# SysCV/sam-pt

Measured on NVIDIA H100. Metric: frames/sec, SAM-PT hot path (PIPS track + SAM ViT encode + prompt/mask decode w/ 12 refinements), higher is better.
Workload: dtype f16 hi.hi + two e4m3 correction passes (~fp32 products) qkv/MLP, f16 hi+lo x3 elsewhere ViT; f32 PIPS + decoder

## Files before the change

### include/sampt_b200.h

```cpp
#ifndef SAMPT_B200_H
#define SAMPT_B200_H
#include <stddef.h>
#include <stdint.h>

#ifdef __cplusplus
extern "C" {
#endif

typedef struct sampt_ctx sampt_ctx;

#define SAMPT_F32 0
#define SAMPT_F16 1
#define SAMPT_U8 2
#define SAMPT_I32 3
#define SAMPT_BF16 4

const char* sampt_last_error(void);
int sampt_version(void);
int sampt_ctx_create(int device, sampt_ctx** out);
int sampt_ctx_destroy(sampt_ctx* ctx);
int sampt_ctx_set_workspace(sampt_ctx* ctx, void* dev_ptr, size_t bytes);
int sampt_ctx_set_vit_workspace(sampt_ctx* ctx, void* dev_ptr, size_t bytes);
int sampt_ctx_set_decoder_workspace(sampt_ctx* ctx, void* dev_ptr, size_t bytes);
int sampt_set_tensor(sampt_ctx* ctx, const char* name, void* dev_ptr, int dtype, int ndim, const int64_t* dims);
int sampt_unset_tensors(sampt_ctx* ctx, const char* prefix);
long long sampt_launch_count(sampt_ctx* ctx);

int sampt_pips_fnet(sampt_ctx* ctx, const uint8_t* frames_u8, int T, int H, int W, int stride, float* fmaps, void* stream);
int sampt_pips_pyramid(sampt_ctx* ctx, const float* fmaps, int T, int H4, int W4, float* l1, float* l2, float* l3,
                       void* stream);
int sampt_pips_track(sampt_ctx* ctx, const float* fmaps, const float* l1, const float* l2, const float* l3, int T, int H4,
                     int W4, const float* query_points, int N, int S, int stride, float thr0, int iters, int flip,
                     int max_windows, float* traj, float* vis, void* stream);
int sampt_pips_window(sampt_ctx* ctx, const float* fmaps, const float* l1, const float* l2, const float* l3, int H4, int W4,
                      const float* xys, const float* coords_init, const float* feat_init, int N, int S, int stride, int iters,
                      float* coords_out, float* vis_e, float* ffeat_out, void* stream);
int sampt_pips_corr_lookup(sampt_ctx* ctx, const float* fmaps, const float* l1, const float* l2, const float* l3, int S,
                           int H4, int W4, const float* ffeats, const float* coords, int N, float* fcorr, void* stream);

int sampt_linear_f32(sampt_ctx* ctx, const float* X, int ldx, const float* W, int ldw, const float* bias,
                     const float* residual, int ldr, float* Y, int ldy, int M, int N, int K, int act, void* stream);

int sampt_gemm_f16(sampt_ctx* ctx, const void* A, int lda, const void* B, int ldb, int M, int N, int K, int precision,
                   int is_bf16, const float* bias, int act, void* out16, float* out32, const float* resid, int ldc,
                   int split_off, void* stream);

int sampt_gemm_f8c(sampt_ctx* ctx, const void* A, const void* B, int M, int N, int K, const float* acc_scale_dev, const float* bias,
                   int act, void* out16, float* out32, const float* resid, int ldc, int split_off, int out_f8, void* stream);
int sampt_split_f8c(sampt_ctx* ctx, const float* x, int M, int K, void* out, void* stream);

int sampt_attention_f16(sampt_ctx* ctx, const void* Qx, const void* Kx, const void* Vt, int BH, int Lq, int Lk, int Lkp, int DK,
                        int HD, int NT, int nheads, void* out, int ld_out, int split_off, void* stream);

int sampt_test_gemm_tc(sampt_ctx* ctx, const void* A, int lda, const void* B, int ldb, int M, int N, int K, int nseg,
                       const int* a_off_host, const int* b_off_host, const int* f8_host, const float* bias, int act, int is_bf16,
                       void* out16, float* out32, const float* resid, int resid_mod, const int* rowmap, const int* skip,
                       const float* acc_scale, int ldc, int split_off, int out_f8, void* stream);
int sampt_test_vit_attention(sampt_ctx* ctx, const void* qkv, const float* rel_pos_h, const float* rel_pos_w, int nwb, int nheads,
                             int S, int D, int DK, int Lkp, void* Qx, void* Kx, void* Vt, void* out, int ld_out, int split_off,
                             int out_f8, void* stream);
int sampt_test_vit_embed(sampt_ctx* ctx, const void* image, int is_f32, int B, int Hr, int Wr, int embed_dim, int img_size,
                         int patch_size, int precision, const float* mean3, const float* std3, void* a_out, float* x_out,
                         void* stream);
int sampt_test_vit_ln(sampt_ctx* ctx, const float* x, int ldx, const int* src, int M, int D, int normalize, const float* gamma,
                      const float* beta, int layout, void* out, void* stream);
int sampt_test_vit_block(sampt_ctx* ctx, int blk, int is_global, float* x, float* x_mid, int B, int Hr, int Wr, int live_only,
                         int embed_dim, int num_heads, int window_size, int img_size, int patch_size, int precision, void* stream);
int sampt_test_vit_neck(sampt_ctx* ctx, const float* x, int B, int embed_dim, int img_size, int patch_size, int out_chans,
                        int precision, float* features, void* stream);
int sampt_test_sam_attention(sampt_ctx* ctx, int kind, const float* q, const float* k, const float* v, float* out, int T, int Nk,
                             void* stream);
int sampt_test_sam_prompt(sampt_ctx* ctx, const float* feat_tok, int G, const float* coords, const int* labels, int K, const float* box,
                          const float* mask_in, float* tokens_out, float* src_out, void* stream);
int sampt_test_sam_upscale(sampt_ctx* ctx, const float* u1, const float* hyper, int n_masks, int G, float* low_res, float* u_out,
                           void* stream);
int sampt_test_sam_postprocess(sampt_ctx* ctx, const float* low_res, int n_masks, int G, int in_h, int in_w, int H, int W, float* out,
                               int* bbox5, float* box4, int* skip, int* n_done, void* stream);
int sampt_test_pips_conv(sampt_ctx* ctx, const char* name, int tc, const void* in, int is_f32, int Nimg, int H, int W, int Cin,
                         int Cout, int R, int stride, int pad, float* out, void* stream);
int sampt_test_pips_inorm(sampt_ctx* ctx, const float* x, const float* res, int mode, int Nimg, int HW, int C, float* y, float* stats,
                          float* res_stats, void* stream);
int sampt_test_pips_resize(sampt_ctx* ctx, const float* in, int Nimg, int Hi, int Wi, int C, float* out, int Ho, int Wo, int Ctot,
                           int coff, void* stream);
int sampt_test_pips_corr(sampt_ctx* ctx, const float* fmaps, const float* l1, const float* l2, const float* l3, int H4, int W4,
                         const float* ffeats, const float* coords, int N, int S, const uint8_t* active_host, int f, int n_missing,
                         const int* slots_host, float* xin, void* stream);
int sampt_test_pips_window_op(sampt_ctx* ctx, int op, int N, int S, int T, int stride, int f, int n_missing, const int* slots_host,
                              const uint8_t* active_host, const float* fmaps, int H4, int W4, float* coords, float* ffeats,
                              float* feat_init, float* traj, float* vis, int* cur, float* x, float* xln, int layer,
                              const float* delta, float thr0, void* stream);
int sampt_test_cotracker_input(sampt_ctx* ctx, const float* fmaps, const float* l1, const float* l2, const float* l3, int H4, int W4,
                               const int* slots_host, const float* coords, const float* ffeats, const float* track_mask,
                               const float* vis_init, const float* time_emb, int N, float* pos, float* xin, void* stream);
int sampt_test_cotracker_ln(sampt_ctx* ctx, int op, const float* x, int M, int K, float* y32, void* y16, void* stream);
int sampt_test_cotracker_attn(sampt_ctx* ctx, const float* qkv, float* out, int G, int L, int gstride, int lstride, int qsplit,
                              void* stream);
int sampt_test_cotracker_block(sampt_ctx* ctx, int kind, int blk, int tc, float* x, int N, void* stream);
int sampt_test_cotracker_update(sampt_ctx* ctx, const float* delta, float* coords, float* ffeats, int N, float* vis_out, void* stream);

int sampt_pil_resize_u8(sampt_ctx* ctx, const uint8_t* in, int B, int H, int W, int Ho, int Wo, const int* hbounds,
                        const int* hcoef, int hksize, const int* vbounds, const int* vcoef, int vksize, uint8_t* tmp,
                        uint8_t* out, void* stream);
int sampt_vit_encode(sampt_ctx* ctx, const uint8_t* resized_u8, int B, int Hr, int Wr, int depth, int embed_dim, int num_heads,
                     int window_size, const int* global_idx_host, int n_global, int img_size, int patch_size, int out_chans,
                     int precision, const float* pixel_mean_host, const float* pixel_std_host, float* features, float* interm,
                     void* stream);

int sampt_sam_features_to_tokens(sampt_ctx* ctx, const float* feat_nchw, float* feat_tok, int C, int GG, void* stream);
int sampt_sam_predict(sampt_ctx* ctx, const float* feat_tok, int G, const float* coords, const int* labels, int K,
                      const float* box, const float* mask_input, int multimask, int in_h, int in_w, int H, int W, float* logits,
// ... 74 lines not shown
```

### sam-pt_b200/csrc/decoder.cu

```cuda
#include <cstdlib>

#include "common.cuh"
#include "kernels.cuh"
#include "tc_api.cuh"
#include "../../include/sampt_b200.h"

namespace sampt {

#define SKIP_RETURN(skip) \
  if ((skip) != nullptr && *(skip) != 0) return;

struct PromptArgs {
  const float* coords;
  const int* labels;
  int K;
  const float* box;
  int use_box;
  const float* gauss;
  const float* pt_emb[4];
  const float* not_a_point;
  const float* out_tokens;
  int n_out_tok;
  float img_size;
};
// ... 729 lines not shown
    SAMPT_TRY(get_f32(c, md + "embedding_encoder.1.weight", &w->enc_lnw)); SAMPT_TRY(get_f32(c, md + "embedding_encoder.1.bias", &w->enc_lnb));
    SAMPT_TRY(get_f32(c, md + "embedding_encoder.3.weight", &w->enc3_w)); SAMPT_TRY(get_f32(c, md + "embedding_encoder.3.bias", &w->enc3_b));
    SAMPT_TRY(get_f32(c, md + "compress_vit_feat.0.weight_gemm", &w->cv0_w)); SAMPT_TRY(get_f32(c, md + "compress_vit_feat.0.bias4", &w->cv0_b4));
    SAMPT_TRY(get_f32(c, md + "compress_vit_feat.1.weight", &w->cv_lnw)); SAMPT_TRY(get_f32(c, md + "compress_vit_feat.1.bias", &w->cv_lnb));
    SAMPT_TRY(get_f32(c, md + "compress_vit_feat.3.weight", &w->cv3_w)); SAMPT_TRY(get_f32(c, md + "compress_vit_feat.3.bias", &w->cv3_b));
    w->vit_dim = (int)c->find(md + "compress_vit_feat.0.weight_gemm")->dims[1];
  }
  return 0;
}

struct DecBufs {
  float *tokens, *queries, *qpe, *tq, *tk, *tv, *ta, *tmp, *mlp_h;
  float *src, *keys, *ik, *iv, *iq, *ia;
  __half *keys16 = nullptr, *ia16 = nullptr;
  float *u1, *hyper, *iou4, *part;
  float *u_sam, *mf1, *mf2;
  int T;
};

#define LAUNCH_OK() do { c->launches++; SAMPT_LAUNCH_CHECK(); } while (0)

static int sg(Ctx* c, cudaStream_t st, const float* X, int ldx, const float* W, const float* b, const float* resid, int ldr,
              float* Y, int ldy, int M, int N, int K, int act, const int* skip) {
  return sgemm_nt_skip(c, st, X, ldx, W, K, b, resid, ldr, Y, ldy, M, N, K, act, skip);
}

__global__ void __launch_bounds__(256)
split_f32_kernel(const float* __restrict__ x, __half* __restrict__ out, long long n4 , int K, const int* skip) {
  SKIP_RETURN(skip);
  const long long i = (long long)blockIdx.x * 256 + threadIdx.x;
  if (i >= n4) return;
  const long long e = i * 4;
  const long long r = e / K;
  const int cidx = (int)(e % K);
  const float4 v = *reinterpret_cast<const float4*>(x + e);
  const __half2 h0 = __floats2half2_rn(v.x, v.y), h1 = __floats2half2_rn(v.z, v.w);
  const float2 f0 = __half22float2(h0), f1 = __half22float2(h1);
  const __half2 l0 = __floats2half2_rn(v.x - f0.x, v.y - f0.y), l1 = __floats2half2_rn(v.z - f1.x, v.w - f1.y);
  __half* o = out + r * 2 * K + cidx;
  *reinterpret_cast<uint2*>(o) = make_uint2(*reinterpret_cast<const uint32_t*>(&h0), *reinterpret_cast<const uint32_t*>(&h1));
  *reinterpret_cast<uint2*>(o + K) = make_uint2(*reinterpret_cast<const uint32_t*>(&l0), *reinterpret_cast<const uint32_t*>(&l1));
}
static int split_rows(Ctx* c, cudaStream_t st, const float* x, __half* out, int rows, int K, const int* skip) {
  const long long n4 = (long long)rows * K / 4;
  split_f32_kernel<<<cdiv(n4, 256), 256, 0, st>>>(x, out, n4, K, skip);
  c->launches++;
  SAMPT_LAUNCH_CHECK();
  return 0;
}
static int tcg(Ctx* c, cudaStream_t st, const __half* X16, const __half* W16, const float* b, const float* resid, float* Y, int ldy,
               int M, int N, int K, const int* skip) {
  GemmSeg seg{};
  seg.nseg = 3;
  seg.a_off[0] = 0; seg.b_off[0] = 0;
  seg.a_off[1] = K; seg.b_off[1] = 0;
  seg.a_off[2] = 0; seg.b_off[2] = K;
  GemmEpi ep{};
  ep.out32 = Y; ep.ldc = ldy; ep.bias = b; ep.resid = resid; ep.skip = skip;
  return gemm_tc(c, st, X16, 2 * K, W16, 2 * K, M, N, K, seg, ep);
}

static int launch_tok_self(Ctx* c, cudaStream_t st, int kind, const float* q, const float* k, const float* v, float* out, int T,
                           const int* skip) {
  if (kind == 1) {
    const size_t smem = ((size_t)2 * T * 33 + (size_t)8 * T + 8 * 32) * sizeof(float);
    SAMPT_CHECK(smem <= 200 * 1024, "too many prompt tokens (%d) for the token self-attention", T);
    SAMPT_TRY(ensure_func_smem(c, "attn_tok_self_kernel<32>", attn_tok_self_kernel<32>, 200 * 1024));
    attn_tok_self_kernel<32><<<dim3(cdiv(T, 32), 8), 256, smem, st>>>(q, k, v, out, T, 8, skip);
  } else {
    attn_q_small_kernel<32><<<dim3(T, 8), 256, 0, st>>>(q, k, v, out, T, 8, skip);
  }
  LAUNCH_OK();
  return 0;
}
static int launch_t2i(Ctx* c, cudaStream_t st, const float* q, const float* k, const float* v, float* part, float* out, int T, int Nk,
                      const int* skip) {
  constexpr int KPS = 256;
  const int nsplit = (Nk + KPS - 1) / KPS;
  attn_t2i_partial_kernel<16, KPS><<<dim3(nsplit, 8), 256, 0, st>>>(q, k, v, part, T, Nk, 8, skip);
  LAUNCH_OK();
  attn_t2i_combine_kernel<16><<<cdiv(T * 128, 128), 128, 0, st>>>(part, out, T, 8, nsplit, skip);
  LAUNCH_OK();
  return 0;
}
static int launch_i2t(Ctx* c, cudaStream_t st, const float* q, const float* k, const float* v, float* out, int N, int T, const int* skip) {
  attn_kv_small_kernel<16><<<cdiv((long long)cdiv(N, 32) * 8, 8), 256, 0, st>>>(q, k, v, out, N, T, 8, skip);
  LAUNCH_OK();
  return 0;
}

static int attn_tok_to_img(Ctx* c, cudaStream_t st, const AttnW& a, const float* q_in, const float* keys, const float* pek,
                           DecBufs& b, float* out , const float* resid, int GG, const int* skip) {
  const int T = b.T;
  SAMPT_TRY(sg(c, st, q_in, 256, a.qw, a.qb, nullptr, 0, b.tq, 128, T, 128, 256, 0, skip));
  if (a.kw16 != nullptr) {
    SAMPT_TRY(tcg(c, st, b.keys16, a.kw16, a.kb, pek, b.ik, 128, GG, 128, 256, skip));
    SAMPT_TRY(tcg(c, st, b.keys16, a.vw16, a.vb, nullptr, b.iv, 128, GG, 128, 256, skip));
  } else {
    SAMPT_TRY(sg(c, st, keys, 256, a.kw, a.kb, pek, 128, b.ik, 128, GG, 128, 256, 0, skip));
    SAMPT_TRY(sg(c, st, keys, 256, a.vw, a.vb, nullptr, 0, b.iv, 128, GG, 128, 256, 0, skip));
  }
  SAMPT_TRY(launch_t2i(c, st, b.tq, b.ik, b.iv, b.part, b.ta, T, GG, skip));
  SAMPT_TRY(sg(c, st, b.ta, 128, a.ow, a.ob, resid, 256, out, 256, T, 256, 128, 0, skip));
  return 0;
}

static int two_way_layer(Ctx* c, cudaStream_t st, const LayerW& L, int idx, DecBufs& b, int GG, const int* skip) {
  const int T = b.T;
  if (idx == 0) {
// ... 493 lines not shown
```

### sam-pt_b200/csrc/gemm_tc.cu

```cuda
#include "common.cuh"
#include "tc_common.cuh"
#include "kernels.cuh"
#include "tc_api.cuh"
#include "../../include/sampt_b200.h"

namespace sampt {

using namespace tc;

constexpr int G_BM = 128, G_BN = 128, G_BK = 64, G_STAGES = 3;
constexpr int G_A_BYTES = G_BM * G_BK * 2;
constexpr int G_B_BYTES = G_BN * G_BK * 2;
constexpr int G_STAGE_BYTES = G_A_BYTES + G_B_BYTES;
constexpr int G_SMEM_BYTES = G_STAGES * G_STAGE_BYTES + 1024  + 256 ;
constexpr int G_THREADS = 288;

__global__ void __launch_bounds__(G_THREADS, 2)
gemm_tc_kernel(const __grid_constant__ CUtensorMap tmA, const __grid_constant__ CUtensorMap tmB, int M, int N, int K,
               GemmSeg seg, GemmEpi ep) {
  if (ep.skip != nullptr && *ep.skip != 0) return;
  extern __shared__ uint8_t smem_raw[];
  uint8_t* smem = reinterpret_cast<uint8_t*>((reinterpret_cast<uintptr_t>(smem_raw) + 1023) & ~uintptr_t(1023));
  uint64_t* full_bar = reinterpret_cast<uint64_t*>(smem + G_STAGES * G_STAGE_BYTES);
  uint64_t* empty_bar = full_bar + G_STAGES;

  const int warp = threadIdx.x >> 5, lane = threadIdx.x & 31;
  const int n_tiles = (N + G_BN - 1) / G_BN;
  const int m_blk = blockIdx.x / n_tiles, n_blk = blockIdx.x % n_tiles;
  int seg_kb[3];
#pragma unroll
  for (int i = 0; i < 3; ++i) seg_kb[i] = i < seg.nseg ? (seg.f8[i] ? K / (2 * G_BK) : K / G_BK) : 0;

  if (threadIdx.x == 0) {
    for (int i = 0; i < G_STAGES; ++i) { mbar_init(&full_bar[i], 1); mbar_init(&empty_bar[i], 256); }
    fence_barrier_init();
  }
  __syncthreads();

  if (warp == 8) {
    if (lane == 0) {
      tma_prefetch_desc(&tmA);
      tma_prefetch_desc(&tmB);
      uint32_t it = 0;
      for (int sg = 0; sg < seg.nseg; ++sg) {
        for (int kb = 0; kb < seg_kb[sg]; ++kb, ++it) {
          const int s = it % G_STAGES;
          const uint32_t ph = (it / G_STAGES) & 1;
          mbar_wait(&empty_bar[s], ph ^ 1);
          const int kk = kb * G_BK;
          uint8_t* sa = smem + s * G_STAGE_BYTES;
          mbar_expect_tx(&full_bar[s], G_STAGE_BYTES);
          tma_load_2d(sa, &tmA, &full_bar[s], seg.a_off[sg] + kk, m_blk * G_BM);
          tma_load_2d(sa + G_A_BYTES, &tmB, &full_bar[s], seg.b_off[sg] + kk, n_blk * G_BN);
        }
      }
    }
    return;
  }

  const int g = warp >> 2, w = warp & 3;
  float acc[64];
#pragma unroll
  for (int i = 0; i < 64; ++i) acc[i] = 0.f;
  uint32_t it = 0;
  int prev_s = -1;
  for (int sg = 0; sg < seg.nseg; ++sg) {
    const bool f8 = seg.f8[sg] != 0;
    for (int kb = 0; kb < seg_kb[sg]; ++kb, ++it) {
      const int s = it % G_STAGES;
      mbar_wait(&full_bar[s], (it / G_STAGES) & 1);
      const uint32_t sa = smem_u32(smem + s * G_STAGE_BYTES);
      const uint64_t adesc = make_smem_desc_sw128(sa + g * 64 * 128);
      const uint64_t bdesc = make_smem_desc_sw128(sa + G_A_BYTES);
      wgmma_fence();
      if (f8) {
#pragma unroll
        for (int k = 0; k < 4; ++k) wgmma_m64n128k32_e4m3(acc, adesc + (uint64_t)(2 * k), bdesc + (uint64_t)(2 * k));
      } else if (ep.is_bf16) {
#pragma unroll
        for (int k = 0; k < 4; ++k) wgmma_m64n128k16_bf16(acc, adesc + (uint64_t)(2 * k), bdesc + (uint64_t)(2 * k));
      } else {
#pragma unroll
        for (int k = 0; k < 4; ++k) wgmma_m64n128k16_f16(acc, adesc + (uint64_t)(2 * k), bdesc + (uint64_t)(2 * k));
      }
      wgmma_commit();
      wgmma_wait<1>();
      if (prev_s >= 0) mbar_arrive(&empty_bar[prev_s]);
      prev_s = s;
    }
  }
  wgmma_wait<0>();
  wgmma_fence_regs(acc);

  const float acc_scale = ep.acc_scale ? __ldg(ep.acc_scale) : 1.0f;
  const int c2 = 2 * (lane & 3);
#pragma unroll
  for (int h = 0; h < 2; ++h) {
    const int m = m_blk * G_BM + g * 64 + w * 16 + (lane >> 2) + 8 * h;
    if (m >= M) continue;
    long long drow = m;
    if (ep.rowmap) drow = ep.rowmap[m];
    if (drow < 0) continue;
#pragma unroll
    for (int i = 0; i < G_BN / 8; ++i) {
      const int n = n_blk * G_BN + 8 * i + c2;
      if (n >= N) continue;
      float v0 = acc[4 * i + 2 * h], v1 = acc[4 * i + 2 * h + 1];
      v0 *= acc_scale; v1 *= acc_scale;
      if (ep.bias) { v0 += __ldg(ep.bias + n); v1 += __ldg(ep.bias + n + 1); }
      if (ep.act == 1) { v0 = gelu_erf(v0); v1 = gelu_erf(v1); }
      else if (ep.act == 3) { v0 = gelu_tanh(v0); v1 = gelu_tanh(v1); }
      if (ep.out32) {
        float* o = ep.out32 + (size_t)drow * ep.ldc + n;
        if (ep.resid) {
          const long long rrow = ep.resid_mod > 0 ? (drow % ep.resid_mod) : drow;
          const float2 t = *reinterpret_cast<const float2*>(ep.resid + (size_t)rrow * ep.ldc + n);
          v0 += t.x; v1 += t.y;
        }
        *reinterpret_cast<float2*>(o) = make_float2(v0, v1);
      } else if (ep.is_bf16) {
        *reinterpret_cast<__nv_bfloat162*>(ep.out16 + (size_t)drow * ep.ldc + n) = __floats2bfloat162_rn(v0, v1);
      } else {
        __half* o = ep.out16 + (size_t)drow * ep.ldc + n;
        const __half2 hv = __floats2half2_rn(v0, v1);
        *reinterpret_cast<__half2*>(o) = hv;
        const float2 hf = __half22float2(hv);
        if (ep.split_off > 0 && ep.out_f8) {
          uint8_t* ob = reinterpret_cast<uint8_t*>(ep.out16 + (size_t)drow * ep.ldc + ep.split_off) + n;
          uint16_t l8, h8;
          asm("cvt.rn.satfinite.e4m3x2.f32 %0, %1, %2;" : "=h"(l8) : "f"((v1 - hf.y) * F8_LO_SCALE), "f"((v0 - hf.x) * F8_LO_SCALE));
          asm("cvt.rn.satfinite.e4m3x2.f32 %0, %1, %2;" : "=h"(h8) : "f"(v1 * F8_HI_SCALE), "f"(v0 * F8_HI_SCALE));
          *reinterpret_cast<uint16_t*>(ob) = l8;
          *reinterpret_cast<uint16_t*>(ob + ep.split_off) = h8;
        } else if (ep.split_off > 0) {
          *reinterpret_cast<__half2*>(o + ep.split_off) = __floats2half2_rn(v0 - hf.x, v1 - hf.y);
        }
      }
    }
  }
}

bool gemm_f8c_applicable(int M, int N, int K) { return M >= 256 && N % 256 == 0 && K % (2 * G_BK) == 0; }

int gemm_tc(Ctx* c, cudaStream_t st, const void* A, int lda, const void* B, int ldb, int M, int N, int K, const GemmSeg& seg,
            const GemmEpi& ep) {
  SAMPT_CHECK(K % G_BK == 0 && K > 0, "gemm_tc: K (%d) must be a positive multiple of %d", K, G_BK);
  SAMPT_CHECK(N % 32 == 0, "gemm_tc: N (%d) must be a multiple of 32", N);
  SAMPT_CHECK(seg.nseg >= 1 && seg.nseg <= 3, "gemm_tc: nseg out of range");
  SAMPT_CHECK((ep.out16 != nullptr) != (ep.out32 != nullptr), "gemm_tc: exactly one of out16/out32 must be set");
  SAMPT_CHECK(ep.ldc % 8 == 0, "gemm_tc: ldc must be a multiple of 8");
  SAMPT_CHECK(ep.act == 0 || ep.act == 1 || ep.act == 3, "gemm_tc: act %d is not 0 (none), 1 (GELU erf) or 3 (GELU tanh)", ep.act);
  const bool f8 = (seg.f8[0] | seg.f8[1] | seg.f8[2]) != 0;
  SAMPT_CHECK(!f8 || K % (2 * G_BK) == 0, "gemm_tc: e4m3 segments need K %% 128 == 0 (K = %d)", K);
  SAMPT_CHECK(!f8 || !ep.is_bf16, "gemm_tc: e4m3 segments go with fp16 operands");
  CUtensorMap tmA, tmB;
  SAMPT_TRY(make_tmap_2d_f16(&tmA, A, (uint64_t)lda, (uint64_t)M, (uint64_t)lda * 2, G_BK, G_BM));
  SAMPT_TRY(make_tmap_2d_f16(&tmB, B, (uint64_t)ldb, (uint64_t)N, (uint64_t)ldb * 2, G_BK, G_BN));
  const int m_tiles = (M + G_BM - 1) / G_BM, n_tiles = (N + G_BN - 1) / G_BN;
  const int grid = m_tiles * n_tiles;
  GemmSeg ord{};
  ord.nseg = seg.nseg;
  int j = 0;
  for (int pass = 1; pass >= 0; --pass)
    for (int i = 0; i < seg.nseg; ++i)
      if ((seg.f8[i] != 0) == (pass == 1)) { ord.a_off[j] = seg.a_off[i]; ord.b_off[j] = seg.b_off[i]; ord.f8[j] = seg.f8[i]; ++j; }
  SAMPT_TRY(ensure_func_smem(c, "gemm_tc_kernel", gemm_tc_kernel, G_SMEM_BYTES));
  gemm_tc_kernel<<<grid, G_THREADS, G_SMEM_BYTES, st>>>(tmA, tmB, M, N, K, ord, ep);
  c->launches++;
  SAMPT_LAUNCH_CHECK();
  return 0;
}

}

using namespace sampt;

extern "C" int sampt_gemm_f16(sampt_ctx* ctx, const void* A, int lda, const void* B, int ldb, int M, int N, int K, int precision,
                              int is_bf16, const float* bias, int act, void* out16, float* out32, const float* resid, int ldc,
                              int split_off, void* stream) {
  Ctx* c = reinterpret_cast<Ctx*>(ctx);
  GemmSeg seg{};
  seg.nseg = precision;
  SAMPT_CHECK(precision >= 1 && precision <= 3, "precision must be 1, 2 or 3");
  if (precision == 2) {
    seg.a_off[0] = 0; seg.b_off[0] = 0;
    seg.a_off[1] = 0; seg.b_off[1] = K;
  } else {
    seg.a_off[0] = 0; seg.b_off[0] = 0;
    seg.a_off[1] = K; seg.b_off[1] = 0;
    seg.a_off[2] = 0; seg.b_off[2] = K;
  }
  GemmEpi ep{};
  ep.out16 = reinterpret_cast<__half*>(out16);
  ep.out32 = out32;
  ep.resid = resid;
  ep.bias = bias;
  ep.rowmap = nullptr;
  ep.ldc = ldc;
  ep.act = act;
  ep.split_off = split_off;
  ep.is_bf16 = is_bf16;
  return gemm_tc(c, reinterpret_cast<cudaStream_t>(stream), A, lda, B, ldb, M, N, K, seg, ep);
}

extern "C" int sampt_gemm_f8c(sampt_ctx* ctx, const void* A, const void* B, int M, int N, int K, const float* acc_scale_dev,
                              const float* bias, int act, void* out16, float* out32, const float* resid, int ldc, int split_off,
                              int out_f8, void* stream) {
  Ctx* c = reinterpret_cast<Ctx*>(ctx);
  SAMPT_CHECK(gemm_f8c_applicable(M, N, K), "sampt_gemm_f8c: needs M >= 256, N %% 256 == 0, K %% 128 == 0 (got %d x %d x %d)", M, N, K);
  GemmEpi ep{};
  ep.out16 = reinterpret_cast<__half*>(out16);
  ep.out32 = out32;
  ep.resid = resid;
  ep.bias = bias;
  ep.ldc = ldc;
  ep.act = act;
  ep.split_off = split_off;
  ep.out_f8 = out_f8;
  ep.acc_scale = acc_scale_dev;
  return gemm_tc(c, reinterpret_cast<cudaStream_t>(stream), A, 2 * K, B, 2 * K, M, N, K, make_seg_f8(K), ep);
}

extern "C" int sampt_test_gemm_tc(sampt_ctx* ctx, const void* A, int lda, const void* B, int ldb, int M, int N, int K, int nseg,
                                  const int* a_off_host, const int* b_off_host, const int* f8_host, const float* bias, int act,
                                  int is_bf16, void* out16, float* out32, const float* resid, int resid_mod, const int* rowmap,
                                  const int* skip, const float* acc_scale, int ldc, int split_off, int out_f8, void* stream) {
  SAMPT_CHECK(nseg >= 1 && nseg <= 3, "sampt_test_gemm_tc: nseg %d out of range", nseg);
  GemmSeg seg{};
  seg.nseg = nseg;
  for (int i = 0; i < nseg; ++i) { seg.a_off[i] = a_off_host[i]; seg.b_off[i] = b_off_host[i]; seg.f8[i] = f8_host[i]; }
  GemmEpi ep{};
  ep.out16 = reinterpret_cast<__half*>(out16);
  ep.out32 = out32;
  ep.resid = resid;
  ep.bias = bias;
  ep.rowmap = rowmap;
  ep.ldc = ldc;
  ep.act = act;
  ep.split_off = split_off;
  ep.is_bf16 = is_bf16;
  ep.resid_mod = resid_mod;
  ep.skip = skip;
  ep.acc_scale = acc_scale;
  ep.out_f8 = out_f8;
  return gemm_tc(reinterpret_cast<Ctx*>(ctx), reinterpret_cast<cudaStream_t>(stream), A, lda, B, ldb, M, N, K, seg, ep);
}

extern "C" int sampt_split_f8c(sampt_ctx* ctx, const float* x, int M, int K, void* out, void* stream) {
  Ctx* c = reinterpret_cast<Ctx*>(ctx);
  return ln_rows(c, reinterpret_cast<cudaStream_t>(stream), x, K, nullptr, nullptr, nullptr, 0.f, reinterpret_cast<__half*>(out), 2 * K, K,
                 M, K, 0, 1);
}
```

### sam-pt_b200/csrc/tc_common.cuh

```cuda
#pragma once
#include <cuda.h>
#include <cuda_runtime.h>
#include <cstdint>

namespace sampt {
namespace tc {

__device__ __forceinline__ uint32_t smem_u32(const void* p) { return (uint32_t)__cvta_generic_to_shared(p); }

__device__ __forceinline__ void mbar_init(uint64_t* bar, uint32_t count) {
  asm volatile("mbarrier.init.shared::cta.b64 [%0], %1;" ::"r"(smem_u32(bar)), "r"(count));
}
__device__ __forceinline__ void fence_barrier_init() { asm volatile("fence.mbarrier_init.release.cluster;" ::: "memory"); }
__device__ __forceinline__ void fence_proxy_async() { asm volatile("fence.proxy.async.shared::cta;" ::: "memory"); }
__device__ __forceinline__ void mbar_expect_tx(uint64_t* bar, uint32_t bytes) {
  asm volatile("mbarrier.arrive.expect_tx.shared::cta.b64 _, [%0], %1;" ::"r"(smem_u32(bar)), "r"(bytes) : "memory");
}
__device__ __forceinline__ void mbar_arrive(uint64_t* bar) {
  asm volatile("mbarrier.arrive.shared::cta.b64 _, [%0];" ::"r"(smem_u32(bar)) : "memory");
}
__device__ __forceinline__ uint32_t mbar_try_wait(uint64_t* bar, uint32_t parity) {
  uint32_t ok;
  asm volatile(
      "{\n"
      ".reg .pred p;\n"
      "mbarrier.try_wait.parity.shared::cta.b64 p, [%1], %2;\n"
      "selp.b32 %0, 1, 0, p;\n"
      "}\n"
      : "=r"(ok)
      : "r"(smem_u32(bar)), "r"(parity)
      : "memory");
  return ok;
}
__device__ __forceinline__ void mbar_wait(uint64_t* bar, uint32_t parity) {
  while (!mbar_try_wait(bar, parity)) {
  }
}

__device__ __forceinline__ void tma_prefetch_desc(const CUtensorMap* m) {
  asm volatile("prefetch.tensormap [%0];" ::"l"(reinterpret_cast<uint64_t>(m)) : "memory");
}
__device__ __forceinline__ void tma_load_2d(void* smem_dst, const CUtensorMap* m, uint64_t* bar, int c0, int c1) {
  asm volatile(
      "cp.async.bulk.tensor.2d.shared::cluster.global.mbarrier::complete_tx::bytes [%0], [%1, {%3, %4}], [%2];" ::"r"(
          smem_u32(smem_dst)),
      "l"(reinterpret_cast<uint64_t>(m)), "r"(smem_u32(bar)), "r"(c0), "r"(c1)
      : "memory");
}
__device__ __forceinline__ void tma_load_3d(void* smem_dst, const CUtensorMap* m, uint64_t* bar, int c0, int c1, int c2) {
  asm volatile(
      "cp.async.bulk.tensor.3d.shared::cluster.global.mbarrier::complete_tx::bytes [%0], [%1, {%3, %4, %5}], [%2];" ::"r"(
          smem_u32(smem_dst)),
      "l"(reinterpret_cast<uint64_t>(m)), "r"(smem_u32(bar)), "r"(c0), "r"(c1), "r"(c2)
      : "memory");
}

__device__ __forceinline__ void wgmma_fence() { asm volatile("wgmma.fence.sync.aligned;" ::: "memory"); }
__device__ __forceinline__ void wgmma_commit() { asm volatile("wgmma.commit_group.sync.aligned;" ::: "memory"); }
template <int N>
__device__ __forceinline__ void wgmma_wait() { asm volatile("wgmma.wait_group.sync.aligned %0;" ::"n"(N) : "memory"); }
template <int R>
__device__ __forceinline__ void wgmma_fence_regs(float (&d)[R]) {
#pragma unroll
  for (int i = 0; i < R; ++i) asm volatile("" : "+f"(d[i])::"memory");
}

__device__ __forceinline__ void wgmma_m64n128k16_f16(float (&d)[64], uint64_t da, uint64_t db) {
  asm volatile(
      "{\n.reg .pred p;\nsetp.ne.b32 p, %66, 0;\n"
      "wgmma.mma_async.sync.aligned.m64n128k16.f32.f16.f16 {%0, %1, %2, %3, %4, %5, %6, %7, %8, %9, %10, %11, %12, %13, %14, %15, %16, %17, %18, %19, %20, %21, %22, %23, %24, %25, %26, %27, %28, %29, %30, %31, %32, %33, %34, %35, %36, %37, %38, %39, %40, %41, %42, %43, %44, %45, %46, %47, %48, %49, %50, %51, %52, %53, %54, %55, %56, %57, %58, %59, %60, %61, %62, %63}, %64, %65, p, 1, 1, 0, 0;\n}\n"
      : "+f"(d[0]), "+f"(d[1]), "+f"(d[2]), "+f"(d[3]), "+f"(d[4]), "+f"(d[5]), "+f"(d[6]), "+f"(d[7]), "+f"(d[8]), "+f"(d[9]), "+f"(d[10]), "+f"(d[11]), "+f"(d[12]), "+f"(d[13]), "+f"(d[14]), "+f"(d[15]), "+f"(d[16]), "+f"(d[17]), "+f"(d[18]), "+f"(d[19]), "+f"(d[20]), "+f"(d[21]), "+f"(d[22]), "+f"(d[23]), "+f"(d[24]), "+f"(d[25]), "+f"(d[26]), "+f"(d[27]), "+f"(d[28]), "+f"(d[29]), "+f"(d[30]), "+f"(d[31]), "+f"(d[32]), "+f"(d[33]), "+f"(d[34]), "+f"(d[35]), "+f"(d[36]), "+f"(d[37]), "+f"(d[38]), "+f"(d[39]), "+f"(d[40]), "+f"(d[41]), "+f"(d[42]), "+f"(d[43]), "+f"(d[44]), "+f"(d[45]), "+f"(d[46]), "+f"(d[47]), "+f"(d[48]), "+f"(d[49]), "+f"(d[50]), "+f"(d[51]), "+f"(d[52]), "+f"(d[53]), "+f"(d[54]), "+f"(d[55]), "+f"(d[56]), "+f"(d[57]), "+f"(d[58]), "+f"(d[59]), "+f"(d[60]), "+f"(d[61]), "+f"(d[62]), "+f"(d[63])
      : "l"(da), "l"(db), "r"(1));
}

__device__ __forceinline__ void wgmma_m64n128k16_bf16(float (&d)[64], uint64_t da, uint64_t db) {
  asm volatile(
      "{\n.reg .pred p;\nsetp.ne.b32 p, %66, 0;\n"
      "wgmma.mma_async.sync.aligned.m64n128k16.f32.bf16.bf16 {%0, %1, %2, %3, %4, %5, %6, %7, %8, %9, %10, %11, %12, %13, %14, %15, %16, %17, %18, %19, %20, %21, %22, %23, %24, %25, %26, %27, %28, %29, %30, %31, %32, %33, %34, %35, %36, %37, %38, %39, %40, %41, %42, %43, %44, %45, %46, %47, %48, %49, %50, %51, %52, %53, %54, %55, %56, %57, %58, %59, %60, %61, %62, %63}, %64, %65, p, 1, 1, 0, 0;\n}\n"
      : "+f"(d[0]), "+f"(d[1]), "+f"(d[2]), "+f"(d[3]), "+f"(d[4]), "+f"(d[5]), "+f"(d[6]), "+f"(d[7]), "+f"(d[8]), "+f"(d[9]), "+f"(d[10]), "+f"(d[11]), "+f"(d[12]), "+f"(d[13]), "+f"(d[14]), "+f"(d[15]), "+f"(d[16]), "+f"(d[17]), "+f"(d[18]), "+f"(d[19]), "+f"(d[20]), "+f"(d[21]), "+f"(d[22]), "+f"(d[23]), "+f"(d[24]), "+f"(d[25]), "+f"(d[26]), "+f"(d[27]), "+f"(d[28]), "+f"(d[29]), "+f"(d[30]), "+f"(d[31]), "+f"(d[32]), "+f"(d[33]), "+f"(d[34]), "+f"(d[35]), "+f"(d[36]), "+f"(d[37]), "+f"(d[38]), "+f"(d[39]), "+f"(d[40]), "+f"(d[41]), "+f"(d[42]), "+f"(d[43]), "+f"(d[44]), "+f"(d[45]), "+f"(d[46]), "+f"(d[47]), "+f"(d[48]), "+f"(d[49]), "+f"(d[50]), "+f"(d[51]), "+f"(d[52]), "+f"(d[53]), "+f"(d[54]), "+f"(d[55]), "+f"(d[56]), "+f"(d[57]), "+f"(d[58]), "+f"(d[59]), "+f"(d[60]), "+f"(d[61]), "+f"(d[62]), "+f"(d[63])
      : "l"(da), "l"(db), "r"(1));
}

__device__ __forceinline__ void wgmma_m64n128k32_e4m3(float (&d)[64], uint64_t da, uint64_t db) {
  asm volatile(
      "{\n.reg .pred p;\nsetp.ne.b32 p, %66, 0;\n"
      "wgmma.mma_async.sync.aligned.m64n128k32.f32.e4m3.e4m3 {%0, %1, %2, %3, %4, %5, %6, %7, %8, %9, %10, %11, %12, %13, %14, %15, %16, %17, %18, %19, %20, %21, %22, %23, %24, %25, %26, %27, %28, %29, %30, %31, %32, %33, %34, %35, %36, %37, %38, %39, %40, %41, %42, %43, %44, %45, %46, %47, %48, %49, %50, %51, %52, %53, %54, %55, %56, %57, %58, %59, %60, %61, %62, %63}, %64, %65, p, 1, 1;\n}\n"
      : "+f"(d[0]), "+f"(d[1]), "+f"(d[2]), "+f"(d[3]), "+f"(d[4]), "+f"(d[5]), "+f"(d[6]), "+f"(d[7]), "+f"(d[8]), "+f"(d[9]), "+f"(d[10]), "+f"(d[11]), "+f"(d[12]), "+f"(d[13]), "+f"(d[14]), "+f"(d[15]), "+f"(d[16]), "+f"(d[17]), "+f"(d[18]), "+f"(d[19]), "+f"(d[20]), "+f"(d[21]), "+f"(d[22]), "+f"(d[23]), "+f"(d[24]), "+f"(d[25]), "+f"(d[26]), "+f"(d[27]), "+f"(d[28]), "+f"(d[29]), "+f"(d[30]), "+f"(d[31]), "+f"(d[32]), "+f"(d[33]), "+f"(d[34]), "+f"(d[35]), "+f"(d[36]), "+f"(d[37]), "+f"(d[38]), "+f"(d[39]), "+f"(d[40]), "+f"(d[41]), "+f"(d[42]), "+f"(d[43]), "+f"(d[44]), "+f"(d[45]), "+f"(d[46]), "+f"(d[47]), "+f"(d[48]), "+f"(d[49]), "+f"(d[50]), "+f"(d[51]), "+f"(d[52]), "+f"(d[53]), "+f"(d[54]), "+f"(d[55]), "+f"(d[56]), "+f"(d[57]), "+f"(d[58]), "+f"(d[59]), "+f"(d[60]), "+f"(d[61]), "+f"(d[62]), "+f"(d[63])
      : "l"(da), "l"(db), "r"(1));
}

// ... 71 lines not shown
```

Before: 23.85.

## Make tensor-core GEMM persistent with ping-pong consumer warpgroups and deeper pipeline

Converts the TMA+wgmma GEMM into a persistent kernel whose grid is capped at the SM count. Two consumer warpgroups alternate whole 128x128 tiles using named barriers, so one warpgroup's epilogue overlaps the other's MMA. When a CTA owns only one tile, the old split across row halves is kept. The pipeline deepens from 3 to 7 stages at one CTA per SM, and the decoder's 3-segment hi/lo order is changed to put the small correction terms first. This aims to hide epilogue cost and cut wave-quantization and launch tail, at the cost of occupancy and more register pressure from the two 64-float accumulators.

```diff
diff --git a/include/sampt_b200.h b/include/sampt_b200.h
--- a/include/sampt_b200.h
+++ b/include/sampt_b200.h
@@ -56,6 +56,11 @@
                        const int* a_off_host, const int* b_off_host, const int* f8_host, const float* bias, int act, int is_bf16,
                        void* out16, float* out32, const float* resid, int resid_mod, const int* rowmap, const int* skip,
                        const float* acc_scale, int ldc, int split_off, int out_f8, void* stream);
+int sampt_test_gemm_tc_grid(sampt_ctx* ctx, const void* A, int lda, const void* B, int ldb, int M, int N, int K, int nseg,
+                            const int* a_off_host, const int* b_off_host, const int* f8_host, const float* bias, int act,
+                            int is_bf16, void* out16, float* out32, const float* resid, int resid_mod, const int* rowmap,
+                            const int* skip, const float* acc_scale, int ldc, int split_off, int out_f8, int max_ctas,
+                            void* stream);
 int sampt_test_vit_attention(sampt_ctx* ctx, const void* qkv, const float* rel_pos_h, const float* rel_pos_w, int nwb, int nheads,
                              int S, int D, int DK, int Lkp, void* Qx, void* Kx, void* Vt, void* out, int ld_out, int split_off,
                              int out_f8, void* stream);
diff --git a/sam-pt_b200/csrc/decoder.cu b/sam-pt_b200/csrc/decoder.cu
--- a/sam-pt_b200/csrc/decoder.cu
+++ b/sam-pt_b200/csrc/decoder.cu
@@ -805,9 +805,9 @@
                int M, int N, int K, const int* skip) {
   GemmSeg seg{};
   seg.nseg = 3;
-  seg.a_off[0] = 0; seg.b_off[0] = 0;
-  seg.a_off[1] = K; seg.b_off[1] = 0;
-  seg.a_off[2] = 0; seg.b_off[2] = K;
+  seg.a_off[0] = K; seg.b_off[0] = 0;
+  seg.a_off[1] = 0; seg.b_off[1] = K;
+  seg.a_off[2] = 0; seg.b_off[2] = 0;
   GemmEpi ep{};
   ep.out32 = Y; ep.ldc = ldy; ep.bias = b; ep.resid = resid; ep.skip = skip;
   return gemm_tc(c, st, X16, 2 * K, W16, 2 * K, M, N, K, seg, ep);
diff --git a/sam-pt_b200/csrc/gemm_tc.cu b/sam-pt_b200/csrc/gemm_tc.cu
--- a/sam-pt_b200/csrc/gemm_tc.cu
+++ b/sam-pt_b200/csrc/gemm_tc.cu
@@ -8,14 +8,144 @@
 
 using namespace tc;
 
-constexpr int G_BM = 128, G_BN = 128, G_BK = 64, G_STAGES = 3;
+constexpr int G_BM = 128, G_BN = 128, G_BK = 64, G_STAGES = 7;
 constexpr int G_A_BYTES = G_BM * G_BK * 2;
 constexpr int G_B_BYTES = G_BN * G_BK * 2;
 constexpr int G_STAGE_BYTES = G_A_BYTES + G_B_BYTES;
 constexpr int G_SMEM_BYTES = G_STAGES * G_STAGE_BYTES + 1024  + 256 ;
-constexpr int G_THREADS = 288;
-
-__global__ void __launch_bounds__(G_THREADS, 2)
+constexpr int G_THREADS = 384;
+constexpr int G_BAR_MMA = 1;
+
+template <int NH>
+__device__ __forceinline__ void gemm_tile_mma(float (&acc)[NH][64], uint8_t* smem, uint64_t* full_bar, uint64_t* empty_bar,
+                                              uint32_t it, const int (&seg_kb)[3], int nseg, const GemmSeg& seg, bool is_bf16,
+                                              int row64, int handoff) {
+#pragma unroll
+  for (int h = 0; h < NH; ++h)
+#pragma unroll
+    for (int i = 0; i < 64; ++i) acc[h][i] = 0.f;
+  int prev_s = -1;
+  for (int sg = 0; sg < nseg; ++sg) {
+    const bool f8 = seg.f8[sg] != 0;
+    for (int kb = 0; kb < seg_kb[sg]; ++kb, ++it) {
+      const int s = it % G_STAGES;
+      mbar_wait(&full_bar[s], (it / G_STAGES) & 1);
+      const uint32_t sa = smem_u32(smem + s * G_STAGE_BYTES);
+      const uint64_t bdesc = make_smem_desc_sw128(sa + G_A_BYTES);
+      uint64_t adesc[NH];
+#pragma unroll
+      for (int h = 0; h < NH; ++h) adesc[h] = make_smem_desc_sw128(sa + (row64 + h) * 64 * 128);
+      wgmma_fence();
+      if (f8) {
+#pragma unroll
+        for (int k = 0; k < 4; ++k)
+#pragma unroll
+          for (int h = 0; h < NH; ++h) wgmma_m64n128k32_e4m3(acc[h], adesc[h] + (uint64_t)(2 * k), bdesc + (uint64_t)(2 * k));
+      } else if (is_bf16) {
+#pragma unroll
+        for (int k = 0; k < 4; ++k)
+#pragma unroll
+          for (int h = 0; h < NH; ++h) wgmma_m64n128k16_bf16(acc[h], adesc[h] + (uint64_t)(2 * k), bdesc + (uint64_t)(2 * k));
+      } else {
+#pragma unroll
+        for (int k = 0; k < 4; ++k)
+#pragma unroll
+          for (int h = 0; h < NH; ++h) wgmma_m64n128k16_f16(acc[h], adesc[h] + (uint64_t)(2 * k), bdesc + (uint64_t)(2 * k));
+      }
+      wgmma_commit();
+      wgmma_wait<1>();
+      if (prev_s >= 0) mbar_arrive(&empty_bar[prev_s]);
+      prev_s = s;
+    }
+  }
+  if (handoff >= 0) named_bar_arrive(handoff, 256);
+  wgmma_wait<0>();
+  mbar_arrive(&empty_bar[prev_s]);
+#pragma unroll
+  for (int h = 0; h < NH; ++h) wgmma_fence_regs(acc[h]);
+}
+
+enum { EPI_F32 = 0, EPI_F16 = 1, EPI_F16_SPLIT = 2, EPI_F16_F8 = 3, EPI_BF16 = 4 };
+
+template <int OUT, int ACT>
+__device__ __forceinline__ void gemm_tile_store(const float (&acc)[64], int m64, int n0, int M, int N, const GemmEpi& ep,
+                                                float acc_scale) {
+  const int w = (threadIdx.x >> 5) & 3, lane = threadIdx.x & 31;
+  const int c2 = 2 * (lane & 3);
+#pragma unroll
+  for (int h = 0; h < 2; ++h) {
+    const int m = m64 + w * 16 + (lane >> 2) + 8 * h;
+    if (m >= M) continue;
+    long long drow = m;
+    if (ep.rowmap) drow = ep.rowmap[m];
+    if (drow < 0) continue;
+#pragma unroll
+    for (int i = 0; i < G_BN / 8; ++i) {
+      const int n = n0 + 8 * i + c2;
+      if (n >= N) continue;
+      float v0 = acc[4 * i + 2 * h], v1 = acc[4 * i + 2 * h + 1];
+      v0 *= acc_scale; v1 *= acc_scale;
+      if (ep.bias) { v0 += __ldg(ep.bias + n); v1 += __ldg(ep.bias + n + 1); }
+      if constexpr (ACT == 1) { v0 = gelu_erf(v0); v1 = gelu_erf(v1); }
+      else if constexpr (ACT == 3) { v0 = gelu_tanh(v0); v1 = gelu_tanh(v1); }
+      if constexpr (OUT == EPI_F32) {
+        float* o = ep.out32 + (size_t)drow * ep.ldc + n;
+        if (ep.resid) {
+          const long long rrow = ep.resid_mod > 0 ? (drow % ep.resid_mod) : drow;
+          const float2 t = *reinterpret_cast<const float2*>(ep.resid + (size_t)rrow * ep.ldc + n);
+          v0 += t.x; v1 += t.y;
+        }
+        *reinterpret_cast<float2*>(o) = make_float2(v0, v1);
+      } else if constexpr (OUT == EPI_BF16) {
+        *reinterpret_cast<__nv_bfloat162*>(ep.out16 + (size_t)drow * ep.ldc + n) = __floats2bfloat162_rn(v0, v1);
+      } else {
+        __half* o = ep.out16 + (size_t)drow * ep.ldc + n;
+        const __half2 hv = __floats2half2_rn(v0, v1);
+        *reinterpret_cast<__half2*>(o) = hv;
+        const float2 hf = __half22float2(hv);
+        if constexpr (OUT == EPI_F16_F8) {
+          uint8_t* ob = reinterpret_cast<uint8_t*>(ep.out16 + (size_t)drow * ep.ldc + ep.split_off) + n;
+          uint16_t l8, h8;
+          asm("cvt.rn.satfinite.e4m3x2.f32 %0, %1, %2;" : "=h"(l8) : "f"((v1 - hf.y) * F8_LO_SCALE), "f"((v0 - hf.x) * F8_LO_SCALE));
+          asm("cvt.rn.satfinite.e4m3x2.f32 %0, %1, %2;" : "=h"(h8) : "f"(v1 * F8_HI_SCALE), "f"(v0 * F8_HI_SCALE));
+          *reinterpret_cast<uint16_t*>(ob) = l8;
+          *reinterpret_cast<uint16_t*>(ob + ep.split_off) = h8;
+        } else if constexpr (OUT == EPI_F16_SPLIT) {
+          *reinterpret_cast<__half2*>(o + ep.split_off) = __floats2half2_rn(v0 - hf.x, v1 - hf.y);
+        }
+      }
+    }
+  }
+}
+
+template <int OUT, int ACT, int NH>
+__device__ __forceinline__ void gemm_tile_store_rows(const float (&acc)[NH][64], int m0, int n0, int M, int N, const GemmEpi& ep,
+                                                     float acc_scale) {
+#pragma unroll
+  for (int h = 0; h < NH; ++h) gemm_tile_store<OUT, ACT>(acc[h], m0 + 64 * h, n0, M, N, ep, acc_scale);
+}
+
+template <int NH>
+__device__ __forceinline__ void gemm_tile_epilogue(const float (&acc)[NH][64], int m0, int n0, int M, int N, const GemmEpi& ep,
+                                                   float acc_scale) {
+  const int out = ep.out32 ? EPI_F32 : ep.is_bf16 ? EPI_BF16 : ep.split_off <= 0 ? EPI_F16 : ep.out_f8 ? EPI_F16_F8 : EPI_F16_SPLIT;
+#define GEMM_EPI_CASE(O)                                                                              \
+  case O:                                                                                             \
+    if (ep.act == 1) gemm_tile_store_rows<O, 1, NH>(acc, m0, n0, M, N, ep, acc_scale);               \
+    else if (ep.act == 3) gemm_tile_store_rows<O, 3, NH>(acc, m0, n0, M, N, ep, acc_scale);          \
+    else gemm_tile_store_rows<O, 0, NH>(acc, m0, n0, M, N, ep, acc_scale);                           \
+    break;
+  switch (out) {
+    GEMM_EPI_CASE(EPI_F32)
+    GEMM_EPI_CASE(EPI_F16)
+    GEMM_EPI_CASE(EPI_F16_SPLIT)
+    GEMM_EPI_CASE(EPI_F16_F8)
+    GEMM_EPI_CASE(EPI_BF16)
+  }
+#undef GEMM_EPI_CASE
+}
+
+__global__ void __launch_bounds__(G_THREADS, 1)
 gemm_tc_kernel(const __grid_constant__ CUtensorMap tmA, const __grid_constant__ CUtensorMap tmB, int M, int N, int K,
                GemmSeg seg, GemmEpi ep) {
   if (ep.skip != nullptr && *ep.skip != 0) return;
@@ -24,126 +154,69 @@
   uint64_t* full_bar = reinterpret_cast<uint64_t*>(smem + G_STAGES * G_STAGE_BYTES);
   uint64_t* empty_bar = full_bar + G_STAGES;
 
-  const int warp = threadIdx.x >> 5, lane = threadIdx.x & 31;
+  const int warp = __shfl_sync(0xffffffffu, (int)threadIdx.x >> 5, 0), lane = threadIdx.x & 31;
   const int n_tiles = (N + G_BN - 1) / G_BN;
-  const int m_blk = blockIdx.x / n_tiles, n_blk = blockIdx.x % n_tiles;
+  const int tiles = ((M + G_BM - 1) / G_BM) * n_tiles;
+  const int my_tiles = (tiles - (int)blockIdx.x + (int)gridDim.x - 1) / (int)gridDim.x;
+  const bool shared_tile = my_tiles == 1;
   int seg_kb[3];
 #pragma unroll
   for (int i = 0; i < 3; ++i) seg_kb[i] = i < seg.nseg ? (seg.f8[i] ? K / (2 * G_BK) : K / G_BK) : 0;
+  const uint32_t tile_kb = seg_kb[0] + seg_kb[1] + seg_kb[2];
 
   if (threadIdx.x == 0) {
-    for (int i = 0; i < G_STAGES; ++i) { mbar_init(&full_bar[i], 1); mbar_init(&empty_bar[i], 256); }
+    for (int i = 0; i < G_STAGES; ++i) { mbar_init(&full_bar[i], 1); mbar_init(&empty_bar[i], shared_tile ? 256 : 128); }
     fence_barrier_init();
   }
   __syncthreads();
 
-  if (warp == 8) {
-    if (lane == 0) {
+  if (warp >= 8) {
+    if (warp == 8 && lane == 0) {
       tma_prefetch_desc(&tmA);
       tma_prefetch_desc(&tmB);
       uint32_t it = 0;
-      for (int sg = 0; sg < seg.nseg; ++sg) {
-        for (int kb = 0; kb < seg_kb[sg]; ++kb, ++it) {
-          const int s = it % G_STAGES;
-          const uint32_t ph = (it / G_STAGES) & 1;
-          mbar_wait(&empty_bar[s], ph ^ 1);
-          const int kk = kb * G_BK;
-          uint8_t* sa = smem + s * G_STAGE_BYTES;
-          mbar_expect_tx(&full_bar[s], G_STAGE_BYTES);
-          tma_load_2d(sa, &tmA, &full_bar[s], seg.a_off[sg] + kk, m_blk * G_BM);
-          tma_load_2d(sa + G_A_BYTES, &tmB, &full_bar[s], seg.b_off[sg] + kk, n_blk * G_BN);
+      for (int t = blockIdx.x; t < tiles; t += gridDim.x) {
+        const int m_blk = t / n_tiles, n_blk = t % n_tiles;
+        for (int sg = 0; sg < seg.nseg; ++sg) {
+          for (int kb = 0; kb < seg_kb[sg]; ++kb, ++it) {
+            const int s = it % G_STAGES;
+            const uint32_t ph = (it / G_STAGES) & 1;
+            mbar_wait(&empty_bar[s], ph ^ 1);
+            const int kk = kb * G_BK;
+            uint8_t* sa = smem + s * G_STAGE_BYTES;
+            mbar_expect_tx(&full_bar[s], G_STAGE_BYTES);
+            tma_load_2d(sa, &tmA, &full_bar[s], seg.a_off[sg] + kk, m_blk * G_BM);
+            tma_load_2d(sa + G_A_BYTES, &tmB, &full_bar[s], seg.b_off[sg] + kk, n_blk * G_BN);
+          }
         }
       }
     }
     return;
   }
 
-  const int g = warp >> 2, w = warp & 3;
-  float acc[64];
-#pragma unroll
-  for (int i = 0; i < 64; ++i) acc[i] = 0.f;
-  uint32_t it = 0;
-  int prev_s = -1;
-  for (int sg = 0; sg < seg.nseg; ++sg) {
-    const bool f8 = seg.f8[sg] != 0;
-    for (int kb = 0; kb < seg_kb[sg]; ++kb, ++it) {
-      const int s = it % G_STAGES;
-      mbar_wait(&full_bar[s], (it / G_STAGES) & 1);
-      const uint32_t sa = smem_u32(smem + s * G_STAGE_BYTES);
-      const uint64_t adesc = make_smem_desc_sw128(sa + g * 64 * 128);
-      const uint64_t bdesc = make_smem_desc_sw128(sa + G_A_BYTES);
-      wgmma_fence();
-      if (f8) {
-#pragma unroll
-        for (int k = 0; k < 4; ++k) wgmma_m64n128k32_e4m3(acc, adesc + (uint64_t)(2 * k), bdesc + (uint64_t)(2 * k));
-      } else if (ep.is_bf16) {
-#pragma unroll
-        for (int k = 0; k < 4; ++k) wgmma_m64n128k16_bf16(acc, adesc + (uint64_t)(2 * k), bdesc + (uint64_t)(2 * k));
-      } else {
-#pragma unroll
-        for (int k = 0; k < 4; ++k) wgmma_m64n128k16_f16(acc, adesc + (uint64_t)(2 * k), bdesc + (uint64_t)(2 * k));
-      }
-      wgmma_commit();
-      wgmma_wait<1>();
-      if (prev_s >= 0) mbar_arrive(&empty_bar[prev_s]);
-      prev_s = s;
-    }
-  }
-  wgmma_wait<0>();
-  wgmma_fence_regs(acc);
-
+  const int g = warp >> 2;
   const float acc_scale = ep.acc_scale ? __ldg(ep.acc_scale) : 1.0f;
-  const int c2 = 2 * (lane & 3);
-#pragma unroll
-  for (int h = 0; h < 2; ++h) {
-    const int m = m_blk * G_BM + g * 64 + w * 16 + (lane >> 2) + 8 * h;
-    if (m >= M) continue;
-    long long drow = m;
-    if (ep.rowmap) drow = ep.rowmap[m];
-    if (drow < 0) continue;
-#pragma unroll
-    for (int i = 0; i < G_BN / 8; ++i) {
-      const int n = n_blk * G_BN + 8 * i + c2;
-      if (n >= N) continue;
-      float v0 = acc[4 * i + 2 * h], v1 = acc[4 * i + 2 * h + 1];
-      v0 *= acc_scale; v1 *= acc_scale;
-      if (ep.bias) { v0 += __ldg(ep.bias + n); v1 += __ldg(ep.bias + n + 1); }
-      if (ep.act == 1) { v0 = gelu_erf(v0); v1 = gelu_erf(v1); }
-      else if (ep.act == 3) { v0 = gelu_tanh(v0); v1 = gelu_tanh(v1); }
-      if (ep.out32) {
-        float* o = ep.out32 + (size_t)drow * ep.ldc + n;
-        if (ep.resid) {
-          const long long rrow = ep.resid_mod > 0 ? (drow % ep.resid_mod) : drow;
-          const float2 t = *reinterpret_cast<const float2*>(ep.resid + (size_t)rrow * ep.ldc + n);
-          v0 += t.x; v1 += t.y;
-        }
-        *reinterpret_cast<float2*>(o) = make_float2(v0, v1);
-      } else if (ep.is_bf16) {
-        *reinterpret_cast<__nv_bfloat162*>(ep.out16 + (size_t)drow * ep.ldc + n) = __floats2bfloat162_rn(v0, v1);
-      } else {
-        __half* o = ep.out16 + (size_t)drow * ep.ldc + n;
-        const __half2 hv = __floats2half2_rn(v0, v1);
-        *reinterpret_cast<__half2*>(o) = hv;
-        const float2 hf = __half22float2(hv);
-        if (ep.split_off > 0 && ep.out_f8) {
-          uint8_t* ob = reinterpret_cast<uint8_t*>(ep.out16 + (size_t)drow * ep.ldc + ep.split_off) + n;
-          uint16_t l8, h8;
-          asm("cvt.rn.satfinite.e4m3x2.f32 %0, %1, %2;" : "=h"(l8) : "f"((v1 - hf.y) * F8_LO_SCALE), "f"((v0 - hf.x) * F8_LO_SCALE));
-          asm("cvt.rn.satfinite.e4m3x2.f32 %0, %1, %2;" : "=h"(h8) : "f"(v1 * F8_HI_SCALE), "f"(v0 * F8_HI_SCALE));
-          *reinterpret_cast<uint16_t*>(ob) = l8;
-          *reinterpret_cast<uint16_t*>(ob + ep.split_off) = h8;
-        } else if (ep.split_off > 0) {
-          *reinterpret_cast<__half2*>(o + ep.split_off) = __floats2half2_rn(v0 - hf.x, v1 - hf.y);
-        }
-      }
-    }
+  if (shared_tile) {
+    const int t = blockIdx.x, m_blk = t / n_tiles, n_blk = t % n_tiles;
+    float acc[1][64];
+    gemm_tile_mma<1>(acc, smem, full_bar, empty_bar, 0, seg_kb, seg.nseg, seg, ep.is_bf16 != 0, g, -1);
+    gemm_tile_epilogue<1>(acc, m_blk * G_BM + g * 64, n_blk * G_BN, M, N, ep, acc_scale);
+    return;
+  }
+  float acc[2][64];
+  for (int i = g; i < my_tiles; i += 2) {
+    const int t = blockIdx.x + i * gridDim.x, m_blk = t / n_tiles, n_blk = t % n_tiles;
+    if (i > 0) named_bar_sync(G_BAR_MMA + g, 256);
+    gemm_tile_mma<2>(acc, smem, full_bar, empty_bar, (uint32_t)i * tile_kb, seg_kb, seg.nseg, seg, ep.is_bf16 != 0, 0,
+                     i + 1 < my_tiles ? G_BAR_MMA + (g ^ 1) : -1);
+    gemm_tile_epilogue<2>(acc, m_blk * G_BM, n_blk * G_BN, M, N, ep, acc_scale);
   }
 }
 
 bool gemm_f8c_applicable(int M, int N, int K) { return M >= 256 && N % 256 == 0 && K % (2 * G_BK) == 0; }
 
-int gemm_tc(Ctx* c, cudaStream_t st, const void* A, int lda, const void* B, int ldb, int M, int N, int K, const GemmSeg& seg,
-            const GemmEpi& ep) {
+static int gemm_tc_launch(Ctx* c, cudaStream_t st, const void* A, int lda, const void* B, int ldb, int M, int N, int K,
+                          const GemmSeg& seg, const GemmEpi& ep, int max_ctas) {
   SAMPT_CHECK(K % G_BK == 0 && K > 0, "gemm_tc: K (%d) must be a positive multiple of %d", K, G_BK);
   SAMPT_CHECK(N % 32 == 0, "gemm_tc: N (%d) must be a multiple of 32", N);
   SAMPT_CHECK(seg.nseg >= 1 && seg.nseg <= 3, "gemm_tc: nseg out of range");
@@ -157,7 +230,8 @@
   SAMPT_TRY(make_tmap_2d_f16(&tmA, A, (uint64_t)lda, (uint64_t)M, (uint64_t)lda * 2, G_BK, G_BM));
   SAMPT_TRY(make_tmap_2d_f16(&tmB, B, (uint64_t)ldb, (uint64_t)N, (uint64_t)ldb * 2, G_BK, G_BN));
   const int m_tiles = (M + G_BM - 1) / G_BM, n_tiles = (N + G_BN - 1) / G_BN;
-  const int grid = m_tiles * n_tiles;
+  int grid = std::min(m_tiles * n_tiles, c->num_sms);
+  if (max_ctas > 0) grid = std::min(grid, max_ctas);
   GemmSeg ord{};
   ord.nseg = seg.nseg;
   int j = 0;
@@ -169,6 +243,11 @@
   c->launches++;
   SAMPT_LAUNCH_CHECK();
   return 0;
+}
+
+int gemm_tc(Ctx* c, cudaStream_t st, const void* A, int lda, const void* B, int ldb, int M, int N, int K, const GemmSeg& seg,
+            const GemmEpi& ep) {
+  return gemm_tc_launch(c, st, A, lda, B, ldb, M, N, K, seg, ep, 0);
 }
 
 }
@@ -221,11 +300,13 @@
   return gemm_tc(c, reinterpret_cast<cudaStream_t>(stream), A, 2 * K, B, 2 * K, M, N, K, make_seg_f8(K), ep);
 }
 
-extern "C" int sampt_test_gemm_tc(sampt_ctx* ctx, const void* A, int lda, const void* B, int ldb, int M, int N, int K, int nseg,
-                                  const int* a_off_host, const int* b_off_host, const int* f8_host, const float* bias, int act,
-                                  int is_bf16, void* out16, float* out32, const float* resid, int resid_mod, const int* rowmap,
-                                  const int* skip, const float* acc_scale, int ldc, int split_off, int out_f8, void* stream) {
+extern "C" int sampt_test_gemm_tc_grid(sampt_ctx* ctx, const void* A, int lda, const void* B, int ldb, int M, int N, int K, int nseg,
+                                       const int* a_off_host, const int* b_off_host, const int* f8_host, const float* bias, int act,
+                                       int is_bf16, void* out16, float* out32, const float* resid, int resid_mod, const int* rowmap,
+                                       const int* skip, const float* acc_scale, int ldc, int split_off, int out_f8, int max_ctas,
+                                       void* stream) {
   SAMPT_CHECK(nseg >= 1 && nseg <= 3, "sampt_test_gemm_tc: nseg %d out of range", nseg);
+  SAMPT_CHECK(max_ctas >= 0, "sampt_test_gemm_tc_grid: max_ctas %d < 0", max_ctas);
   GemmSeg seg{};
   seg.nseg = nseg;
   for (int i = 0; i < nseg; ++i) { seg.a_off[i] = a_off_host[i]; seg.b_off[i] = b_off_host[i]; seg.f8[i] = f8_host[i]; }
@@ -243,7 +324,16 @@
   ep.skip = skip;
   ep.acc_scale = acc_scale;
   ep.out_f8 = out_f8;
-  return gemm_tc(reinterpret_cast<Ctx*>(ctx), reinterpret_cast<cudaStream_t>(stream), A, lda, B, ldb, M, N, K, seg, ep);
+  return gemm_tc_launch(reinterpret_cast<Ctx*>(ctx), reinterpret_cast<cudaStream_t>(stream), A, lda, B, ldb, M, N, K, seg, ep,
+                        max_ctas);
+}
+
+extern "C" int sampt_test_gemm_tc(sampt_ctx* ctx, const void* A, int lda, const void* B, int ldb, int M, int N, int K, int nseg,
+                                  const int* a_off_host, const int* b_off_host, const int* f8_host, const float* bias, int act,
+                                  int is_bf16, void* out16, float* out32, const float* resid, int resid_mod, const int* rowmap,
+                                  const int* skip, const float* acc_scale, int ldc, int split_off, int out_f8, void* stream) {
+  return sampt_test_gemm_tc_grid(ctx, A, lda, B, ldb, M, N, K, nseg, a_off_host, b_off_host, f8_host, bias, act, is_bf16, out16,
+                                 out32, resid, resid_mod, rowmap, skip, acc_scale, ldc, split_off, out_f8, 0, stream);
 }
 
 extern "C" int sampt_split_f8c(sampt_ctx* ctx, const float* x, int M, int K, void* out, void* stream) {
diff --git a/sam-pt_b200/csrc/tc_common.cuh b/sam-pt_b200/csrc/tc_common.cuh
--- a/sam-pt_b200/csrc/tc_common.cuh
+++ b/sam-pt_b200/csrc/tc_common.cuh
@@ -36,6 +36,9 @@
   while (!mbar_try_wait(bar, parity)) {
   }
 }
+
+__device__ __forceinline__ void named_bar_sync(int id, int count) { asm volatile("bar.sync %0, %1;" ::"r"(id), "r"(count) : "memory"); }
+__device__ __forceinline__ void named_bar_arrive(int id, int count) { asm volatile("bar.arrive %0, %1;" ::"r"(id), "r"(count) : "memory"); }
 
 __device__ __forceinline__ void tma_prefetch_desc(const CUtensorMap* m) {
   asm volatile("prefetch.tensormap [%0];" ::"l"(reinterpret_cast<uint64_t>(m)) : "memory");
```

Result: faster. 26.65 (median of 6 runs) (+11.8%).
